# StanfordASL/GuSTO.jl

Hardware: AMD Instinct MI355X
Metric: converged trajectories/sec (batched SCP), freeflyer_se2 N=50, inputs resident in HBM (higher is better)
Workload: dtype f64

## Files before the change

gusto.jl_amd/csrc/common.hpp:

```cpp
#pragma once
#include <hip/hip_runtime.h>
#include <math.h>
#include <stdint.h>

#include "gusto_hip.h"

namespace gusto {

#define GD __device__ __forceinline__
typedef double v4d __attribute__((ext_vector_type(4)));

constexpr int ROW_HARD = 0;
constexpr int ROW_PEN = 1;
constexpr int ROW_PEN_TR = 2;
constexpr int ROW_PEN_EQ = 3;
constexpr int ROW_HARD_EQ = 4;
constexpr int ROW_EQ = 5;
GD bool row_is_hard(int kind) { return kind == ROW_HARD || kind == ROW_HARD_EQ; }

constexpr int RS_T = 0, RS_LAM = 1, RS_LAMB = 2, RS_S = 3, RS_DT = 4, RS_DL = 5, RS_DS = 6, RS_KA = 7, RS_KB = 8,
              RS_NVAR = 9;

#ifndef GUSTO_DUBINS_WAVES
#define GUSTO_DUBINS_WAVES 2
#endif
#ifndef GUSTO_WAVES_PER_EU
#define GUSTO_WAVES_PER_EU 1
#endif

#ifndef GUSTO_TO_SWEEP_CALL
#define GUSTO_TO_SWEEP_CALL true
#endif
#ifndef GUSTO_TO4_SWEEP_CALL
// ... 3 lines not shown
#define GUSTO_SWEEP_DPP 1
#endif
#ifndef GUSTO_FACTOR_LDS
#define GUSTO_FACTOR_LDS 1
#endif
#ifndef GUSTO_FACTOR_LDS_MV
#define GUSTO_FACTOR_LDS_MV 1
#endif
#ifndef GUSTO_FACTOR_LDS_HUU
#define GUSTO_FACTOR_LDS_HUU 0
#endif
#ifndef GUSTO_FACTOR_LDS_ROWS
#define GUSTO_FACTOR_LDS_ROWS 1
#endif
#ifndef GUSTO_FACTOR_HUU_DPP
#define GUSTO_FACTOR_HUU_DPP 0
#endif
#ifndef GUSTO_FACTOR_LAZY_SINV
#define GUSTO_FACTOR_LAZY_SINV 1
#endif
#ifndef GUSTO_FACTOR_LAZY_D
#define GUSTO_FACTOR_LAZY_D 1
#endif
static_assert(!(GUSTO_FACTOR_LDS_HUU && GUSTO_FACTOR_HUU_DPP), "H_uu to the Cholesky through LDS or by DPP, not both");
static_assert(!GUSTO_FACTOR_LAZY_D || GUSTO_FACTOR_LAZY_SINV, "GUSTO_FACTOR_LAZY_D forms D from the L^-1 that GUSTO_FACTOR_LAZY_SINV stores");
#ifndef GUSTO_USE_MFMA
#define GUSTO_USE_MFMA true
#endif
constexpr int GUSTO_TO_FREEFLYER_SE2 = 4, GUSTO_TO_ASTROBEE_SE3 = 5, GUSTO_TO_ASTROBEE_SE3_MANIFOLD = 6;
constexpr double TRAJOPT_DEFECT_REG = 1e-4;
constexpr int RS_EARLIER = 0, RS_ROW = 1, RS_ROW_LANE = 2;
template <int MODEL> struct MT;
template <> struct MT<GUSTO_FREEFLYER_SE2> {
    static constexpr int NDEF = 0;
    static constexpr int n = 6, m = 3, WS = 2, NFIX = 3, NHU = 2;
    static constexpr int WAVES_PER_EU = GUSTO_WAVES_PER_EU;
    static constexpr int RS_FORM = RS_ROW;
    static constexpr bool SWEEP_CALL = false;
    static constexpr bool SWEEP_DPP = GUSTO_SWEEP_DPP;
    static constexpr bool FACTOR_LDS = GUSTO_FACTOR_LDS;
    static constexpr bool FACTOR_REC = true;
    static constexpr bool MFMA = false;
    static constexpr int SCHED_PROBE = 2;
    static constexpr int SCHED_SLICE = 4;
    static constexpr bool LTI = true, HAS_OBS = true;
    static constexpr bool PG2 = true;
    static constexpr int pg_r0(int c) { return c < 3 ? c : (c < 6 ? c - 3 : c - 6); }
    static constexpr int pg_r1(int c) { return c < 3 ? c + 3 : (c < 6 ? c : c - 3); }
    static constexpr bool Anz(int i, int j) { return j == i + 3; }
    static constexpr bool Mnz(int i, int j) { return i == j || j == i + 3; }
    static constexpr bool Bnz(int i, int j) { return i == j + 3; }
    static constexpr bool Gnz(int i, int j) { return i == j || i == j + 3; }
    static constexpr bool Hnz(int, int) { return true; }
};
template <> struct MT<GUSTO_DUBINS_CAR> {
    static constexpr int NDEF = 0;
    static constexpr int n = 3, m = 1, WS = 2, NFIX = 6, NHU = 2;
    static constexpr int WAVES_PER_EU = GUSTO_DUBINS_WAVES;
    static constexpr int RS_FORM = RS_ROW;
    static constexpr bool SWEEP_CALL = false;
// ... 155 lines not shown
        for (int i2 = 0; i2 < n; i2++)
            for (int l2 = 0; l2 < n; l2++)
                if (T::Mnz(l2, i2) && (i2 < i || (i2 == i && l2 < l))) c++;
        return c;
    }
    static constexpr int NPHI = pos_phi(0, n);
    static constexpr int pos_gam(int l, int j) {
        int c = NPHI;
        for (int l2 = 0; l2 < n; l2++)
            for (int j2 = 0; j2 < m; j2++)
                if (T::Gnz(l2, j2) && (l2 < l || (l2 == l && j2 < j))) c++;
        return c;
    }
    static constexpr int NS = pos_gam(n, 0);
    static constexpr int S = (NS + 15) / 16 * 16;
    static constexpr bool USE = T::MFMA && T::NDEF == 0;
};

template <int MODEL> constexpr int rs_stride_rt(int N) { return MT<MODEL>::RS_FORM == RS_EARLIER ? N : (N + 63) & ~63; }
template <int MODEL, bool ONE> GD int rs_stride(int N) {
    if constexpr (ONE && MT<MODEL>::RS_FORM != RS_EARLIER) return 64;
    else return rs_stride_rt<MODEL>(N);
}
template <int MODEL, bool ONE> constexpr int rs_form() { return (ONE && MT<MODEL>::RS_FORM == RS_ROW_LANE) ? RS_ROW : MT<MODEL>::RS_FORM; }

struct WsLayout {
    int nslot;
    size_t rowstate, obs_nh, obs_c0, obs_mask, PG, PGS, QQ, Paft, Piaft, KD, Phicl, pvt, to_traj, total;
};
template <int MODEL> inline WsLayout make_ws_layout(int N, int n_obs) {
    using T = MT<MODEL>;
    constexpr int n = T::n, m = T::m, NZ = n + m;
    WsLayout L;
    L.nslot = T::NFIX + n_obs + 2 * n + T::NHU;
    size_t o = 0;
    auto take = [&](size_t c) { size_t r = o; o += (c + 1) & ~size_t(1); return r; };
    L.rowstate = take((size_t)RS_NVAR * L.nslot * rs_stride_rt<MODEL>(N));
    L.obs_nh = take((size_t)n_obs * T::WS * N);
    L.obs_c0 = take((size_t)n_obs * N);
    L.obs_mask = take((size_t)N);
    L.PG = take((size_t)(T::LTI ? 1 : N) * n * NZ);
    L.PGS = take(SpPG<MODEL>::USE ? (size_t)N * SpPG<MODEL>::S : 0);
    using R = Rec<MODEL>;
    L.QQ = take((size_t)N * R::SQQ);
    L.Paft = take((size_t)(N + 1) * R::SNN) + R::SNN;
    L.Piaft = take((size_t)(N + 1) * R::SNN) + R::SNN;
    L.KD = take((size_t)N * R::SKD);
// ... 451 lines not shown
```

gusto.jl_amd/csrc/ipm.hpp:

```cpp
#pragma once
#include "rows.hpp"

#ifndef GUSTO_COOP_CHOL_MIN
#define GUSTO_COOP_CHOL_MIN 7
#endif

namespace gusto {

extern __shared__ __attribute__((aligned(16))) double gusto_dyn_lds[];

template <int MODEL> constexpr bool costate_adjoint();

struct IpmOut {
    int status, iters;
    double obj, res_p, res_d, mu;
};

template <bool ONEWAVE> GD void blk_sync() {
    if constexpr (ONEWAVE) {
#ifdef GUSTO_STRICT_SYNC
        asm volatile("s_waitcnt vmcnt(0) lgkmcnt(0)\n\ts_barrier" ::: "memory");
#endif
        __builtin_amdgcn_fence(__ATOMIC_ACQ_REL, "wavefront");
        __builtin_amdgcn_wave_barrier();
// ... 318 lines not shown
                    for (int l = 0; l < n; l++) if (T::Bnz(l, j)) s += M[i * n + l] * (h * B[l * m + j]);
                    const double v = knot0 ? h * B[i * m + j] : 2.0 * s;
                    pg[i * NZ + n + j] = v;
                    if constexpr (SPR) if (T::Gnz(i, j)) ps[SP::pos_gam(i, j)] = v;
                }
                if constexpr (T::NDEF > 0) {
#pragma unroll
                    for (int j = 0; j < T::NDEF; j++) pg[i * NZ + n + (m - T::NDEF) + j] = (i == j) ? 1.0 : 0.0;
                }
            }
        }
        uint64_t mask = 0;
        if constexpr (T::HAS_OBS) {
            double xw[T::WS];
#pragma unroll
            for (int j = 0; j < T::WS; j++) xw[j] = xp[j];
            const Env E = K.env();
            for (int i = 0; i < E.n_obs; i++) {
                double nh[T::WS];
                const double dist = signed_distance<T::WS>(K.P, E, 0, xw, i, nh);
                if (dist < toggle) {
                    mask |= (uint64_t)1 << i;
                    double c0 = K.P.mp.clearance - dist;
#pragma unroll
                    for (int j = 0; j < T::WS; j++) {
                        K.obs_nh[((size_t)i * T::WS + j) * K.N + k] = nh[j];
                        c0 += nh[j] * xw[j];
                    }
                    K.obs_c0[(size_t)i * K.N + k] = c0;
                }
            }
        }
        K.obs_mask[k] = mask;
    }
    K.sync();
}

template <int MODEL, class BLK> GD void factor_sweep_mw(BLK& K, double* fail, Prof& pf) {
    using T = MT<MODEL>;
    using R = Rec<MODEL>;
    constexpr int n = T::n, m = T::m, NZ = n + m, NQ = NZ * (NZ + 1) / 2, NPG = n * NZ;
    constexpr int QPT = (NQ + 63) / 64, PPT = (NPG + 63) / 64;
    const int tid = K.tid, NT = K.nt(), N = K.N;
    for (int e = tid; e < n * n; e += NT) { K.sP[e] = 0; K.sPi[e] = 0; K.sGd[e] = 0; }
    double qq[QPT], pgn[PPT];
#pragma unroll
// ... 1776 lines not shown
        RowPre<NP> pre;
        if constexpr (NP > 0) {
            const int slot_u = RowSlots<MODEL>::ctl(K.P.n_obs);
            pre.load(rs, T::NFIX, slot_u, [&](int var) {
                return var == RS_T || var == RS_LAM || var == RS_S || var == RS_LAMB || (pass && (var == RS_KA || var == RS_KB));
            });
        }
        double hdx[ADJ ? n : 1];
#pragma unroll
        for (int i = 0; i < (ADJ ? n : 1); i++) hdx[i] = 0;
        OpStep<NP, ADJ, RS> op{rs, dxs, dus, pass, mu_t, tau, gAx, gAu, gBx, gBu, &pre, hdx};
        ctx.tick(0);
#if GUSTO_SEG_W2
        if constexpr (NCH > 0) {
            const bool cs = pass == 1 || ncomp == 0;
            segw_post_rows<MODEL, NCH>(K, cs ? SEGW_STEP_CS : SEGW_STEP, (double)pass, ctx.kappa, ctx.omega, ctx.Delta, mu_t, tau);
            RowCtx<MODEL> cm = ctx;
            cm.mask = (cs && NCH == 2) ? (cm.mask & seg_obs_share(0, 2)) : 0;
            visit_rows<MODEL>(cm, xs, us, op);
            segw_join();
            segw_rows_step_add<MODEL, NCH>(K.lds, K.P.ll.seg, k, (cs && NCH > 2) ? 1 : 0, op, gAx, gBx);
        } else
#endif
        visit_rows<MODEL>(ctx, xs, us, op);
        ctx.tick(3);
        if constexpr (ADJ) {
            if (adj_rt && k >= 1 && (pass == 1 || ncomp == 0)) {
                double Mk[n * n], Gamk[n * m], w[n];
                load_M_Gam(K, k, Mk, Gamk);
#pragma unroll
                for (int i = 0; i < n; i++) {
                    double s = hdx[i] + (pass ? K.gAx_(k, i) + mu_t * K.gBx_(k, i) : 0.0);
                    if (k == N - 1 && K.is_goal(i)) s += mugn[i];
                    w[i] = s;
                }
#pragma unroll
                for (int i = 0; i < n; i++) {
                    double s = 0;
#pragma unroll
                    for (int l = 0; l < n; l++) if (T::Mnz(l, i)) s += Mk[l * n + i] * w[l];
                    K.nun[k * n + i] = s;
                }
            }
        }
        l_amax = op.amax.value(); l_c0 = op.c0; l_c1 = op.c1; l_c2 = op.c2;
        if (pass == 0) {
#pragma unroll
// ... 85 lines not shown
        constexpr int NP = (n <= 8 && T::NDEF == 0) ? T::NFIX + T::NHU : 0;
        RowPre<NP> pre;
        if constexpr (NP > 0) {
            const int slot_u = RowSlots<MODEL>::ctl(K.P.n_obs);
            const bool upd = alpha_prev != 0.0;
            pre.load(rs, T::NFIX, slot_u, [&](int var) {
                return var == RS_T || var == RS_LAM || var == RS_S || var == RS_LAMB ||
                       (upd && (var == RS_DT || var == RS_DL || var == RS_DS));
            });
        }
        constexpr bool LRTR = MODEL == GUSTO_ASTROBEE_SE3;
        OpResidHess<n, m, NP, LRTR, RS> op{rs, Hx, Hu, rdx, rdu, gx0, gu0, alpha_prev, &pre};
        ctx.tick(0);
#if GUSTO_SEG_W2
        if constexpr (NCH > 0) {
            segw_post_rows<MODEL, NCH>(K, SEGW_ROWS_R, alpha_prev, ctx.kappa, ctx.omega, ctx.Delta, 0.0, 0.0);
            RowCtx<MODEL> cm = ctx;
            cm.mask = 0;
            visit_rows<MODEL>(cm, xs, us, op);
            segw_join();
            segw_rows_resid_add<MODEL, NCH>(K.lds, K.P.ll.seg, k, NCH - 1, op, Hx, rdx, gx0);
        } else
#endif
        visit_rows<MODEL>(ctx, xs, us, op);
        ctx.tick(3);
#pragma unroll
        for (int i = 0; i < n; i++) K.dXs_(k, i) = gx0[i];
#pragma unroll
        for (int i = 0; i < m; i++) K.dUs_(k, i) = gu0[i];
        l_comp = op.comp;
        l_resp = nanmax(l_resp, op.maxrp);
#pragma unroll
        for (int i = 0; i < m; i++) {
            const double wi_ = (i < m - T::NDEF) ? wk : TRAJOPT_DEFECT_REG * wk;
            Hu[sidx(i, i, m)] += 2 * wi_; rdu[i] += 2 * wi_ * us[i];
        }
        {
            double vs[n], vd[n];
#pragma unroll
            for (int i = 0; i < n; i++) {
                const double n1 = (k + 1 < N) ? K.nu[(k + 1) * n + i] : 0.0, n0 = (k >= 1) ? K.nu[k * n + i] : 0.0;
                vs[i] = n1 + n0; vd[i] = n1 - n0;
                l_numax = fmax(l_numax, fabs(K.nu[k * n + i]));
            }
#pragma unroll
            for (int i = 0; i < n; i++) {
                double s = vd[i];
// ... 154 lines not shown
    RS rs{K.rowstate, K.P.wl.nslot, rs_stride<MODEL, BLK::ONE>(N), act ? k : 0};
#define GUSTO_REFRESH_K()                                     \
    do {                                                      \
        asm volatile("" : "+v"(k));                           \
        ctx.k = k; rs.k = act ? k : 0;                        \
        ctx.xp = K.Xp + (act ? k : 0) * n;                    \
    } while (0)

    auto load_iter = [&](double* xs, double* us) {
#pragma unroll
        for (int i = 0; i < n; i++) xs[i] = K.Xw[k * n + i];
#pragma unroll
        for (int i = 0; i < m; i++) us[i] = K.Uw[k * m + i];
    };

    double ncomp_l = 0;
    if (act) {
        double xs[n], us[m];
#pragma unroll
        for (int i = 0; i < n; i++) { xs[i] = (k == 0) ? K.x_init[i] : K.Xp[k * n + i]; K.Xw[k * n + i] = xs[i]; K.nu[k * n + i] = 0; }
#pragma unroll
        for (int i = 0; i < m; i++) { us[i] = K.Up[k * m + i]; K.Uw[k * m + i] = us[i]; }
        OpInit<RS> op{rs, muw};
        visit_rows<MODEL>(ctx, xs, us, op);
        ncomp_l = op.ncomp;
    }
    if (k == 0) {
        *fail = 0.0;
        for (int i = 0; i < n; i++) { mug[i] = 0; mugn[i] = 0; }
    }
    const double ncomp = block_reduce<BLK::ONE>(ncomp_l, OpSum(), red);
    K.sync();
    pf.tick(PF_INIT);

    constexpr bool LINC = BLK::C::LC_LDS;
    if constexpr (LINC) {
        if (act) {
            double xpk[n], c2[2];
#pragma unroll
            for (int i = 0; i < n; i++) xpk[i] = K.Xp[k * n + i];
            Dyn<MODEL>::lin_cache(K.P.mp, xpk, c2);
            K.lcl[2 * k] = c2[0]; K.lcl[2 * k + 1] = c2[1];
        }
        K.sync();
    }
    int status = GUSTO_SOLVER_FAILED, it = 0, n_acc = 0;
    bool adj_ok = true;
// ... 240 lines not shown
                xs[i] += alpha * K.dXs_(k, i);
                K.Xw[k * n + i] = xs[i];
                K.nu[k * n + i] += alpha * (K.nun[k * n + i] - K.nu[k * n + i]);
            }
#pragma unroll
            for (int i = 0; i < m; i++) { us[i] += alpha * K.dUs_(k, i); K.Uw[k * m + i] = us[i]; }
        }
        alpha_prev = alpha;
        if constexpr (n > 4) {
            if (k < n) mug[k] += alpha * (mugn[k] - mug[k]);
        } else if (k == 0) {
            for (int i = 0; i < n; i++) mug[i] += alpha * (mugn[i] - mug[i]);
        }
        K.sync();
        pf.tick(PF_UPDATE);
    }
    double l_obj = 0;
    if (act) {
        double xs[n], us[m];
        load_iter(xs, us);
#pragma unroll
        for (int i = 0; i < m; i++) l_obj += ((i < m - T::NDEF) ? wk : TRAJOPT_DEFECT_REG * wk) * us[i] * us[i];
        OpSlackSum<RS> op{rs};
        visit_rows<MODEL>(ctx, xs, us, op);
        l_obj += op.sum;
    }
    const double obj = block_reduce<BLK::ONE>(l_obj, OpSum(), red);
    K.sync();
#undef GUSTO_REFRESH_K
    out.status = status; out.iters = it; out.obj = obj / kappa; out.res_p = res_p; out.res_d = res_d; out.mu = mu;
}

}
```

gusto.jl_amd/csrc/launch.hpp:

```cpp
#pragma once
#include <algorithm>
#include <cstdlib>
#include <cstdio>
#include <cstring>

#include "handle.hpp"
#include "scp.hpp"

using namespace gusto;

#ifdef GUSTO_DEV_KNOBS
static inline const char* dev_env(const char* k) { return getenv(k); }
#else
static inline const char* dev_env(const char*) { return nullptr; }
#endif

static inline int launch_waves(gusto_handle h) {
    int w = h->waves;
    if (const char* e = dev_env("GUSTO_DEV_WAVES")) w = atoi(e);
    const int need = (h->N + 63) / 64;
    return std::min(4, std::max(w, need));
}
template <int MODEL> static int fill_params(gusto_handle h, KParams& P, int B, bool need_env = true) {
    using T = MT<MODEL>;
    memset(&P, 0, sizeof(P));
    P.N = h->N; P.B = B; P.n_fresh = B;
    if (!fill_env(h, P, T::HAS_OBS, need_env)) {
        h->err = "gusto_set_env_batch described a different number of problems than gusto_set_problems";
        return GUSTO_ERR_STATE;
    }
    P.hist_cap = h->hist_cap;
    P.sp = h->sp; P.mp = h->mp; P.io = h->io;
    warm_defaults(MODEL, P.io);
    P.X = h->d_X; P.U = h->d_U;
    P.x_init = h->d_xinit; P.goal_lo = h->d_glo; P.goal_hi = h->d_ghi; P.tf = h->d_tf;
    P.sub_Delta = h->d_subD; P.sub_omega = h->d_subW; P.sub_toggle = h->d_subT; P.sub_X = h->d_subX; P.sub_U = h->d_subU;
    P.sub_obj = h->d_subObj; P.sub_status = h->d_subSt; P.sub_iters = h->d_subIt;
    P.st_i = h->d_sti; P.st_d = h->d_std;
    P.J_true = h->d_Jt; P.J_full = h->d_Jf; P.conv = h->d_conv; P.Delta = h->d_Delta; P.omega = h->d_omega; P.rho = h->d_rho;
    P.accept = h->d_acc; P.scp_status = h->d_scp; P.solver_status = h->d_sol; P.tr_sat = h->d_tr; P.cvx_sat = h->d_cvx;
    P.ipm_it = h->d_ipm;
    P.tp = h->tp; P.to_mu = h->d_to_mu; P.to_xtol = h->d_to_xtol; P.to_ftol = h->d_to_ftol; P.to_ctol = h->d_to_ctol;
    P.wl = make_ws_layout<MODEL>(h->N, P.n_obs);
    P.ll = make_lds_layout<MODEL>(h->N, launch_waves(h) > (h->N + 63) / 64);
    HIPCHK(h, h->d_queue.alloc(SQ_WORDS));
#ifdef GUSTO_PROFILE
    HIPCHK(h, h->d_prof.alloc((size_t)h->batch_cap * PROF_N));
#endif
    P.prof = h->d_prof;
    return GUSTO_OK;
}

template <class Kern, class Pre>
static int enqueue_solve(gusto_handle h, KParams& P, Kern kern, dim3 grid, dim3 block, size_t lds, Pre pre) {
    HIPCHK(h, h->d_ws.ensure(P.wl.total * (size_t)grid.x));
    P.ws = h->d_ws;
    HIPCHK(h, hipEventRecord(h->ev0, h->stream));
    { int rc = pre(); if (rc) return rc; }
    hipLaunchKernelGGL(kern, grid, block, lds, h->stream, P);
    HIPCHK(h, hipGetLastError());
    HIPCHK(h, hipEventRecord(h->ev1, h->stream));
    h->sched_err = 0;
    HIPCHK(h, gusto_fetch_sched_err(h));
    h->pending = true;
    return GUSTO_OK;
}

template <int MODEL> static int launch_scp(gusto_handle h, int mode, int max_iter, int force) {
    using T = MT<MODEL>;
    KParams P;
    int rc = fill_params<MODEL>(h, P, h->B);
    if (rc) return rc;
    P.mode = mode; P.max_iter = max_iter; P.force = force;
    const int NT = 64 * launch_waves(h);
    size_t lds = (size_t)P.ll.total * sizeof(double);
    if (const char* pad = dev_env("GUSTO_DEV_LDS_KB")) lds = std::max(lds, (size_t)atoi(pad) * 1024);
    if (lds > 160 * 1024) { h->err = "problem does not fit the 160 KiB LDS of a CU"; return GUSTO_ERR_ARG; }
    auto kern = (NT == 64) ? &scp_kernel<MODEL, true> : &scp_kernel<MODEL, false>;
    int per_cu = 0, cus = 0;
// ... 109 lines not shown
```

gusto.jl_amd/csrc/rows.hpp:

```cpp
#pragma once
#include <type_traits>

#include "models.hpp"

namespace gusto {

#ifndef GUSTO_OBS_BATCH
#define GUSTO_OBS_BATCH 4
#endif
constexpr int OBS_BATCH = GUSTO_OBS_BATCH, FX_OBS = 64;

template <int CNT> struct RowEv {
    double g;
    double raw;
    double gr[CNT];
    double hd[CNT];
};

template <int MODEL> struct RowCtx {
    const KParams* P;
    int N, k, nslot;
    double kappa, omega, Delta;
    GPtr<const double> xp;
    uint64_t mask;
// ... 38 lines not shown
template <bool ISU, int I0, int CNT, int FX = -1, class Op>
GD void lin_row(Op& op, int slot, int kind, const double* v, const double* b, double c0, double mul, double off) {
    RowEv<CNT> ev;
    double g = c0;
#pragma unroll
    for (int j = 0; j < CNT; j++) {
        g += b[j] * v[I0 + j];
        ev.gr[j] = mul * b[j];
        ev.hd[j] = 0.0;
    }
    ev.raw = g;
    ev.g = mul * g - off;
    op.template row<ISU, I0, CNT, FX>(slot, kind, ev);
}

template <int MODEL> struct RowSlots {
    using T = MT<MODEL>;
    static constexpr bool CT = T::RS_FORM != RS_EARLIER;
    GD static int ctl(int n_obs) { return CT ? T::NFIX : T::NFIX + n_obs + 2 * T::n; }
    GD static int goal(int n_obs) { return CT ? T::NFIX + T::NHU : T::NFIX + n_obs; }
    GD static int obs(int n_obs) { return CT ? T::NFIX + T::NHU + 2 * T::n : T::NFIX; }
};

template <int MODEL, class Op> GD void visit_obs_rows(const RowCtx<MODEL>& c, const double* xs, Op& op, uint64_t mk) {
    using T = MT<MODEL>;
    const double kw = c.kappa * c.omega;
    const int slot_obs = RowSlots<MODEL>::obs(c.P->n_obs);
    while (mk) {
        int oi[OBS_BATCH], oslot[OBS_BATCH];
        bool ov[OBS_BATCH];
        int last = 0;
#pragma unroll
        for (int q = 0; q < OBS_BATCH; q++) {
            ov[q] = mk != 0;
            if (ov[q]) { last = __ffsll((unsigned long long)mk) - 1; mk &= mk - 1; }
            oi[q] = last; oslot[q] = slot_obs + last;
        }
        double ob[OBS_BATCH][T::WS], oc[OBS_BATCH];
#pragma unroll
        for (int q = 0; q < OBS_BATCH; q++) {
#pragma unroll
            for (int j = 0; j < T::WS; j++) ob[q][j] = -(c.obs_nh + (size_t)(oi[q] * T::WS + j) * (size_t)c.N)[c.k];
            oc[q] = (c.obs_c0 + (size_t)oi[q] * (size_t)c.N)[c.k];
        }
        op.obs_load(oslot);
        static_for<0, OBS_BATCH>([&](auto Q) {
            constexpr int q = decltype(Q)::value;
            if (ov[q]) lin_row<false, 0, T::WS, FX_OBS + q>(op, oslot[q], ROW_PEN, xs, ob[q], oc[q], kw, 0.0);
        });
    }
}

template <int MODEL, class Op> GD void visit_ctl_rows(const RowCtx<MODEL>& c, const double* us, Op& op) {
    using T = MT<MODEL>;
    constexpr int n = T::n;
    constexpr bool is2 = MODEL == GUSTO_FREEFLYER_SE2, FB = Op::FIX_BATCH;
    const gusto_model_params& mp = c.P->mp;
    const int slot_u = RowSlots<MODEL>::ctl(c.P->n_obs);
    if (c.k < c.N - 1) {
        constexpr int nf = is2 ? 2 : 3, im = is2 ? 2 : 3, nm = is2 ? 1 : 3;
        double af[nf], am[nm];
#pragma unroll
        for (int j = 0; j < nf; j++) af[j] = 1.0 / (mp.mass * mp.mass);
#pragma unroll
        for (int j = 0; j < nm; j++) { const double ji = 1.0 / mp.Jdiag[is2 ? 2 : j]; am[j] = ji * ji; }
        if constexpr (FB) {
            int fs[OBS_BATCH];
#pragma unroll
            for (int q = 0; q < OBS_BATCH; q++) fs[q] = slot_u + (q < 1 ? 0 : 1);
            op.obs_load(fs);
        }
        quad_row<true, 0, nf, (FB ? FX_OBS + 0 : T::NFIX)>(op, slot_u, ROW_HARD, us, af, nullptr, -mp.hard_limit_accel * mp.hard_limit_accel,
                              1.0 / (mp.hard_limit_accel * mp.hard_limit_accel), 0.0);
        quad_row<true, im, nm, (FB ? FX_OBS + 1 : T::NFIX + 1)>(op, slot_u + 1, ROW_HARD, us, am, nullptr, -mp.hard_limit_alpha * mp.hard_limit_alpha,
                               1.0 / (mp.hard_limit_alpha * mp.hard_limit_alpha), 0.0);
    }
}

template <int MODEL, class Op> GD void visit_rows(const RowCtx<MODEL>& c, const double* xs, const double* us, Op& op) {
    using T = MT<MODEL>;
    constexpr int n = T::n;
    const gusto_model_params& mp = c.P->mp;
    const double kw = c.kappa * c.omega;
    const int slot_obs = RowSlots<MODEL>::obs(c.P->n_obs), slot_goal = RowSlots<MODEL>::goal(c.P->n_obs), slot_u = RowSlots<MODEL>::ctl(c.P->n_obs);
    double one[n];
#pragma unroll
    for (int j = 0; j < n; j++) one[j] = 1.0;

    if constexpr (T::NDEF > 0) {
        constexpr bool is2 = MODEL == GUSTO_TO_FREEFLYER_SE2, man = MODEL == GUSTO_TO_ASTROBEE_SE3_MANIFOLD;
        constexpr int nv = is2 ? 2 : 3, iw = is2 ? 5 : (man ? 10 : 9), nw = is2 ? 1 : 3, m0 = T::m - T::NDEF;
        constexpr bool FB = Op::FIX_BATCH;
#define GUSTO_FXQ(q) (FB ? FX_OBS + (q) : -1)
        auto batch = [&](int s0, int s1, int s2, int s3) {
            if constexpr (FB) { const int fs[OBS_BATCH] = {s0, s1, s2, s3}; op.obs_load(fs); }
        };
        static_assert(OBS_BATCH == 4 || !FB, "batches of four rows");
        if constexpr (!man) {
            batch(0, 1, 2, 2);
            quad_row<false, 0, n, GUSTO_FXQ(0)>(op, 0, ROW_HARD, xs, one, c.xp, -c.Delta, 1.0 / c.Delta, 0.0);
        } else {
            const double* qp = c.xp + 6;
// ... 80 lines not shown
#define GUSTO_FXB(i, fx) ((FB && (i) < NB1) ? FX_OBS + (i) : (fx))
        if constexpr (FB) {
            int fs[OBS_BATCH];
#pragma unroll
            for (int q = 0; q < OBS_BATCH; q++) fs[q] = q < NB1 ? q : NB1 - 1;
            op.obs_load(fs);
        }
        if constexpr (!man) {
            quad_row<false, 0, n, GUSTO_FXB(0, 0)>(op, slot++, ROW_PEN_TR, xs, one, c.xp, 0.0, kw, c.kappa * c.Delta);
        } else {
            const double* qp = c.xp + 6;
            const double qn = sqrt(qp[0] * qp[0] + qp[1] * qp[1] + qp[2] * qp[2] + qp[3] * qp[3]);
            double bp[4], bm[4], c0 = qn - 1.0;
#pragma unroll
            for (int j = 0; j < 4; j++) { bp[j] = qp[j] / qn; bm[j] = -bp[j]; c0 -= qp[j] * qp[j] / qn; }
            lin_row<false, 6, 4, GUSTO_FXB(0, 0)>(op, slot++, ROW_HARD_EQ, xs, bm, -c0, kw, c.kappa * c.P->sp.eps);
            lin_row<false, 6, 4, GUSTO_FXB(1, 1)>(op, slot++, ROW_PEN_EQ, xs, bp, c0, kw, c.kappa * c.P->sp.eps);
            const double m1 = -1.0;
            lin_row<false, 6, 1, GUSTO_FXB(2, 2)>(op, slot++, ROW_PEN, xs, &m1, 0.0, kw, 0.0);
        }
        quad_row<false, 3, nv, GUSTO_FXB(T::NFIX - 2, T::NFIX - 2)>(op, slot++, ROW_PEN, xs, one, nullptr, -mp.hard_limit_vel * mp.hard_limit_vel, kw, 0.0);
        quad_row<false, iw, nw, GUSTO_FXB(T::NFIX - 1, T::NFIX - 1)>(op, slot++, ROW_PEN, xs, one, nullptr, -mp.hard_limit_omega * mp.hard_limit_omega, kw, 0.0);
        c.tick(1);
        visit_obs_rows<MODEL>(c, xs, op, c.mask);
        c.tick(2);
        if (!c.skip_ctl) visit_ctl_rows<MODEL>(c, us, op);
#undef GUSTO_FXB
    } else {
        static_for<0, n>([&](auto I) {
            constexpr int i = decltype(I)::value;
            const double p1 = 1.0, m1 = -1.0;
            lin_row<false, i, 1, i>(op, i, ROW_PEN, xs, &p1, -mp.x_max[i], kw, 0.0);
            lin_row<false, i, 1, n + i>(op, n + i, ROW_PEN, xs, &m1, mp.x_min[i], kw, 0.0);
        });
        if (c.k < c.N - 1) {
            const double p1 = 1.0, m1 = -1.0;
            lin_row<true, 0, 1, T::NFIX>(op, slot_u, ROW_HARD, us, &p1, -mp.u_max, 1.0 / fabs(mp.u_max), 0.0);
            lin_row<true, 0, 1, T::NFIX + 1>(op, slot_u + 1, ROW_HARD, us, &m1, mp.u_min, 1.0 / fabs(mp.u_min), 0.0);
        }
    }
    if (c.boxmask != 0 && c.k == c.N - 1) {
        static_assert(OBS_BATCH >= 4, "a batch holds the four rows of two coordinates");
        static_for<0, (n + 1) / 2>([&](auto G) {
            constexpr int i0 = 2 * decltype(G)::value, i1 = (i0 + 1 < n) ? i0 + 1 : i0;
            if ((c.boxmask >> i0) & 3u) {
                const double lo0 = c.goal_lo[i0], hi0 = c.goal_hi[i0], lo1 = c.goal_lo[i1], hi1 = c.goal_hi[i1];
                int oslot[OBS_BATCH];
#pragma unroll
                for (int q = 0; q < OBS_BATCH; q++) oslot[q] = slot_goal + 2 * ((q < 2) ? i0 : i1) + (q & 1);
                op.obs_load(oslot);
                const double p1 = 1.0, m1 = -1.0;
                if (lo0 != hi0) {
                    const double hw = (isfinite(hi0) && isfinite(lo0)) ? 0.5 * (hi0 - lo0) : 1.0;
                    const double sc = 1.0 / fmax(1e-3, fmin(1.0, hw));
                    if (isfinite(hi0)) lin_row<false, i0, 1, FX_OBS + 0>(op, oslot[0], ROW_HARD, xs, &p1, -hi0, sc, 0.0);
                    if (isfinite(lo0)) lin_row<false, i0, 1, FX_OBS + 1>(op, oslot[1], ROW_HARD, xs, &m1, lo0, sc, 0.0);
                }
                if (i1 != i0 && lo1 != hi1) {
                    const double hw = (isfinite(hi1) && isfinite(lo1)) ? 0.5 * (hi1 - lo1) : 1.0;
                    const double sc = 1.0 / fmax(1e-3, fmin(1.0, hw));
                    if (isfinite(hi1)) lin_row<false, i1, 1, FX_OBS + 2>(op, oslot[2], ROW_HARD, xs, &p1, -hi1, sc, 0.0);
                    if (isfinite(lo1)) lin_row<false, i1, 1, FX_OBS + 3>(op, oslot[3], ROW_HARD, xs, &m1, lo1, sc, 0.0);
                }
            }
        });
    }
}

template <int FORM> struct RowState {
    GPtr<double> base;
    int nslot, kp, k;
    GD auto& at(int var, int slot) const {
        if constexpr (FORM == RS_EARLIER) return (base + (size_t)(var * nslot + slot) * (size_t)kp)[k];
        else {
            typedef __attribute__((address_space(1))) char GC;
            typedef __attribute__((address_space(1))) double GV;
            const int mid = FORM == RS_ROW_LANE ? var : RS_NVAR / 2;
            GC* r = (GC*)base.p + (size_t)(((unsigned)(slot * RS_NVAR + mid) * (unsigned)kp + (unsigned)k) * 8u);
            return *(GV*)(r + (ptrdiff_t)((var - mid) * kp) * 8);
        }
    }
};

template <int NP> struct RowPre {
    double v[RS_NVAR][NP > 0 ? NP : 1];
    template <class RS, class F> GD void load(const RS& rs, int nfix, int slot_u, F&& want) {
#pragma unroll
        for (int var = 0; var < RS_NVAR; var++)
#pragma unroll
            for (int i = 0; i < NP; i++)
                if (want(var)) v[var][i] = rs.at(var, i < nfix ? i : slot_u + (i - nfix));
    }
};

struct ObsPre {
    double v[RS_NVAR][OBS_BATCH];
    template <class RS, class F> GD void load(const RS& rs, const int* slot, F&& want) {
#pragma unroll
        for (int var = 0; var < RS_NVAR; var++)
            if (want(var)) {
#pragma unroll
                for (int q = 0; q < OBS_BATCH; q++) v[var][q] = rs.at(var, slot[q]);
            }
    }
};

template <class RS> struct OpInit {
    static constexpr bool FIX_BATCH = false;
    RS rs;
    double muw;
    int ncomp = 0;
    GD void obs_load(const int*) {}
    template <bool ISU, int I0, int CNT, int FX> GD void row(int slot, int kind, const RowEv<CNT>& ev) {
        if (kind == ROW_EQ) {
            rs.at(RS_T, slot) = 1.0; rs.at(RS_LAM, slot) = 0.0; rs.at(RS_LAMB, slot) = 0.0; rs.at(RS_S, slot) = 0.0;
        } else if (row_is_hard(kind)) {
            const double t = fmax(-ev.g, 1e-2), mu0 = (muw > 0) ? muw : 0.01;
            rs.at(RS_T, slot) = t; rs.at(RS_LAM, slot) = mu0 / t; rs.at(RS_LAMB, slot) = 0.0; rs.at(RS_S, slot) = 0.0;
            ncomp += 1;
        } else if (muw > 0) {
            const double g = ev.g, ag = fabs(g), rr = sqrt(g * g + 4 * muw * muw);
            const double big = muw + 0.5 * (rr + ag), small = muw + 2 * muw * muw / (rr + ag);
            const double s = (g >= 0) ? big : small, t = (g >= 0) ? small : big;
            rs.at(RS_S, slot) = s; rs.at(RS_T, slot) = t; rs.at(RS_LAM, slot) = muw / t; rs.at(RS_LAMB, slot) = muw / s;
            ncomp += 2;
        } else {
            const double s = fmax(ev.g, 0.0) + 0.01;
            rs.at(RS_S, slot) = s; rs.at(RS_T, slot) = s - ev.g; rs.at(RS_LAM, slot) = 0.5; rs.at(RS_LAMB, slot) = 0.5;
            ncomp += 2;
        }
    }
};

template <int n, int m, int NP, bool LRTR, class RS> struct OpResidHess {
    static constexpr bool FIX_BATCH = NP == 0;
    RS rs;
// ... 2 lines not shown
    const RowPre<NP>* pre;
    double comp = 0, maxrp = 0;
    ObsPre ob;
    double trs = 0, trg[LRTR ? n : 1], trh[LRTR ? n : 1];
    GD void obs_load(const int* slot) {
        const bool upd = alpha_prev != 0.0;
        ob.load(rs, slot, [&](int var) {
            return var == RS_T || var == RS_LAM || var == RS_S || var == RS_LAMB ||
                   (upd && (var == RS_DT || var == RS_DL || var == RS_DS));
        });
    }
    template <int FX> GD double get(int var, int slot) const {
        if constexpr (FX >= FX_OBS) return ob.v[var][FX - FX_OBS];
        else if constexpr (FX >= 0 && NP > 0) return pre->v[var][FX];
        else return rs.at(var, slot);
    }
    template <bool ISU, int I0, int CNT, int FX> GD void row(int slot, int kind, const RowEv<CNT>& ev) {
        double t = get<FX>(RS_T, slot), lam = get<FX>(RS_LAM, slot);
        double sig, rp;
        if (alpha_prev != 0.0) {
            const double dl = get<FX>(RS_DL, slot);
            t += alpha_prev * get<FX>(RS_DT, slot);
            lam += alpha_prev * dl;
            rs.at(RS_T, slot) = t; rs.at(RS_LAM, slot) = lam;
        }
        if (kind == ROW_EQ) {
            rp = ev.g;
            sig = 1.0 / TRAJOPT_EQ_DELTA;
        } else if (row_is_hard(kind)) {
            rp = ev.g + t;
            comp += t * lam;
            sig = lam * rcp_nr(t);
        } else {
            double s = get<FX>(RS_S, slot), lamb = get<FX>(RS_LAMB, slot);
            if (alpha_prev != 0.0) {
                s += alpha_prev * get<FX>(RS_DS, slot);
                lamb -= alpha_prev * get<FX>(RS_DL, slot);
                rs.at(RS_S, slot) = s; rs.at(RS_LAMB, slot) = lamb;
            }
            rp = ev.g - s + t;
            comp += t * lam + s * lamb;
            sig = lam * lamb * rcp_nr(t * lamb + lam * s);
        }
        maxrp = nanmax(maxrp, fabs(rp));
        double* H = ISU ? Hu : Hx;
        double* r = ISU ? rdu : rdx;
        double* g0 = ISU ? gu0 : gx0;
        const double coef0 = lam + sig * ev.g;
        constexpr int dim = ISU ? m : n;
        if constexpr (LRTR && !ISU && CNT == n) {
            trs = sig;
#pragma unroll
            for (int a = 0; a < CNT; a++) {
                r[I0 + a] += lam * ev.gr[a];
                g0[I0 + a] += coef0 * ev.gr[a];
                trg[a] = ev.gr[a];
                trh[a] = lam * ev.hd[a];
            }
            return;
        }
#pragma unroll
// ... 29 lines not shown
    StepFrac amax;
    double c0 = 0, c1 = 0, c2 = 0;
    ObsPre ob;
    GD void obs_load(const int* slot) {
        ob.load(rs, slot, [&](int var) {
            return var == RS_T || var == RS_LAM || var == RS_S || var == RS_LAMB || (pass && (var == RS_KA || var == RS_KB));
        });
    }
    template <int FX> GD double get(int var, int slot) const {
        if constexpr (FX >= FX_OBS) return ob.v[var][FX - FX_OBS];
        else if constexpr (FX >= 0 && NP > 0) return pre->v[var][FX];
        else return rs.at(var, slot);
    }
    template <bool ISU, int I0, int CNT, int FX> GD void row(int slot, int kind, const RowEv<CNT>& ev) {
        const double t = get<FX>(RS_T, slot), lam = get<FX>(RS_LAM, slot);
        const double ka = pass ? get<FX>(RS_KA, slot) : 0.0;
        const double* dv = ISU ? dus : dxs;
        double w = 0;
#pragma unroll
        for (int a = 0; a < CNT; a++) w += ev.gr[a] * dv[I0 + a];
        double dt, dl, ds;
        double cA = 0, cB = 0;
        double sig = 0;
        if (kind == ROW_EQ) {
            sig = 1.0 / TRAJOPT_EQ_DELTA;
            dl = sig * (ev.g + w);
            if constexpr (HDX && !ISU) {
                const double sw = sig * w;
#pragma unroll
                for (int a = 0; a < CNT; a++) hdx[I0 + a] += sw * ev.gr[a];
            }
            if (pass == 0) {
                rs.at(RS_KA, slot) = 0.0;
                const double cE = lam + sig * ev.g;
                double* gA = ISU ? gAu : gAx;
#pragma unroll
                for (int a = 0; a < CNT; a++) gA[I0 + a] += cE * ev.gr[a];
            }
            if (pass) { rs.at(RS_DT, slot) = 0.0; rs.at(RS_DL, slot) = dl; rs.at(RS_DS, slot) = 0.0; }
            return;
        }
        if (row_is_hard(kind)) {
            const double rp = ev.g + t;
            const double rt = rcp_nr(t);
            dt = -rp - w;
            dl = (mu_t - t * lam - ka - lam * dt) * rt;
            ds = 0.0;
            if (pass == 0) { cA = (lam * rp - dt * dl) * rt; cB = rt; }
            if constexpr (HDX) sig = lam * rt;
        } else {
            const double s = get<FX>(RS_S, slot), lamb = get<FX>(RS_LAMB, slot);
            const double kb = pass ? get<FX>(RS_KB, slot) : 0.0;
            const double rp = ev.g - s + t;
            const double il = rcp_nr(lamb), lol = lam * il;
            const double D = t + lol * s;
            const double rho0 = mu_t - t * lam - ka + lam * rp - lol * (mu_t - s * lamb - kb);
            const double rD = rcp_nr(D);
            dl = (rho0 + lam * w) * rD;
            ds = (mu_t - s * lamb - kb + s * dl) * il;
            dt = -rp - w + ds;
            if constexpr (HDX) sig = lam * rD;
            amax.test(s, ds, tau);
            amax.test(lamb, -dl, tau);
            if (pass == 0) {
                c0 += s * lamb; c1 += ds * lamb - s * dl; c2 -= ds * dl; rs.at(RS_KB, slot) = -ds * dl;
                cA = lam + (lam * rp - t * lam - dt * dl + lol * (s * lamb - ds * dl)) * rD;
                cB = (1.0 - lol) * rD;
            }
        }
        if constexpr (HDX && !ISU) {
            const double sw = sig * w;
#pragma unroll
            for (int a = 0; a < CNT; a++) hdx[I0 + a] += sw * ev.gr[a] + (lam * ev.hd[a]) * dv[I0 + a];
        }
        amax.test(t, dt, tau);
        amax.test(lam, dl, tau);
        if (pass == 0) {
            c0 += t * lam; c1 += dt * lam + t * dl; c2 += dt * dl; rs.at(RS_KA, slot) = dt * dl;
            double* gA = ISU ? gAu : gAx;
            double* gB = ISU ? gBu : gBx;
#pragma unroll
            for (int a = 0; a < CNT; a++) { gA[I0 + a] += cA * ev.gr[a]; gB[I0 + a] += cB * ev.gr[a]; }
        }
        if (pass) { rs.at(RS_DT, slot) = dt; rs.at(RS_DL, slot) = dl; rs.at(RS_DS, slot) = ds; }
    }
};

template <class RS> struct OpSlackSum {
    static constexpr bool FIX_BATCH = false;
    RS rs;
    double sum = 0;
    GD void obs_load(const int*) {}
    template <bool ISU, int I0, int CNT, int FX> GD void row(int slot, int kind, const RowEv<CNT>&) {
        if (!row_is_hard(kind) && kind != ROW_EQ) sum += rs.at(RS_S, slot);
    }
};

struct OpCheck {
    static constexpr bool FIX_BATCH = false;
    double eps;
    bool ok = true;
    GD void obs_load(const int*) {}
    template <bool ISU, int I0, int CNT, int FX> GD void row(int, int kind, const RowEv<CNT>& ev) {
        if (ISU) return;
        if (kind == ROW_PEN && ev.raw >= eps) ok = false;
        if (kind == ROW_PEN_EQ && (ev.raw <= -eps || ev.raw >= eps)) ok = false;
// ... 5 lines not shown
```

gusto.jl_amd/csrc/scp.hpp:

```cpp
#pragma once
#include "ipm.hpp"

#ifndef GUSTO_WAVES_PER_EU
#define GUSTO_WAVES_PER_EU 1
#endif

namespace gusto {

template <class BLK> GD double cost_true(BLK& K, const double* U) {
    constexpr int m = BLK::m, mc = m - BLK::T::NDEF;
    const int k = K.tid;
    double l = 0;
    if (k >= 1 && k < K.N) {
#pragma unroll
        for (int j = 0; j < mc; j++) l += 0.5 * K.dt * (U[(k - 1) * m + j] * U[(k - 1) * m + j] + U[k * m + j] * U[k * m + j]);
    }
    return block_reduce<BLK::ONE>(l, OpSum(), K.misc);
}

template <int MODEL, class BLK> GD double trust_region_ratio(BLK& K, const double* X, const double* U, const double* Xp, const double* Up) {
    using T = MT<MODEL>;
    constexpr int n = T::n, m = T::m;
    const int k = K.tid, N = K.N;
    double num = 0, den = 0;
// ... 105 lines not shown
        const int h = n_hist;
        if (tid == 0) { P.solver_status[hb + h] = io.status; P.ipm_it[hb + h] = io.iters; }
        if (io.status != GUSTO_SOLVER_OPTIMAL && io.status != GUSTO_SOLVER_ALMOST) {
            stop = GUSTO_STOP_SUBPROBLEM_FAILED;
            break;
        }
        double dn = 0, xn = 0;
        bool cvx_l = true;
        if (k < N) {
            double xs[n], us[m];
#pragma unroll
            for (int i = 0; i < n; i++) {
                xs[i] = K.Xw[k * n + i];
                const double e = xs[i] - K.Xp[k * n + i];
                dn += e * e; xn += xs[i] * xs[i];
            }
#pragma unroll
            for (int i = 0; i < m; i++) us[i] = K.Uw[k * m + i];
            RowCtx<MODEL> ctx;
            ctx.P = &P; ctx.N = N; ctx.k = k; ctx.nslot = P.wl.nslot; ctx.kappa = 1.0; ctx.omega = 1.0; ctx.Delta = 1.0;
            ctx.xp = K.Xp + k * n; ctx.mask = K.obs_mask[k]; ctx.obs_nh = K.obs_nh; ctx.obs_c0 = K.obs_c0;
            ctx.goal_lo = K.goal_lo; ctx.goal_hi = K.goal_hi; ctx.boxmask = K.boxmask;
            OpCheck op{sp.eps};
            visit_rows<MODEL>(ctx, xs, us, op);
            cvx_l = op.ok;
        }
        tk(1);
        const double max_d2 = block_reduce<ONEWAVE>(dn, OpMax(), K.misc);
        const double max_x2 = block_reduce<ONEWAVE>(xn, OpMax(), K.misc);
        const double conv = sqrt(max_d2) / sqrt(max_x2);
        const int cvx_sat = block_reduce<ONEWAVE>(cvx_l ? 0.0 : 1.0, OpMax(), K.misc) == 0.0;
        tk(2);
        const int tr_sat = (max_d2 - Delta <= P.io.tr_tol * fmax(1.0, Delta));
        int accept, status;
        double Delta_n, omega_n;
        if (tr_sat) {
            const double rho = trust_region_ratio<MODEL>(K, K.Xw, K.Uw, K.Xp, K.Up);
            tk(3);
            if (tid == 0) P.rho[hb + n_rho] = rho;
            n_rho++;
            if (rho > sp.rho1) {
                status = GUSTO_SCP_INACCURATE_MODEL; accept = 0; Delta_n = sp.beta_fail * Delta; omega_n = omega;
            } else {
                accept = 1;
                Delta_n = (rho < sp.rho0) ? fmin(sp.beta_succ * Delta, sp.Delta0) : Delta;
                if (!cvx_sat) { status = GUSTO_SCP_VIOLATES_CONSTRAINTS; omega_n = sp.gamma_fail * omega; }
                else { status = GUSTO_SCP_OK; omega_n = omega; }
// ... 464 lines not shown
```

Before: 151,900.

## Interleave row-state variables into 16-byte pairs for wide global loads/stores

Adds an RS_PAIR row-state layout for single-wave blocks that interleaves related IPM variables (t/lam, s/lamb, dt/dl, ka/kb) so each pair is read or written with one 16-byte vector access. All row-state accessors (init, residual, step, prefetch) gain pair paths, and KB is now stored together with KA. An optional paired obstacle-normal layout is added but disabled by default. Alignment checks are added at launch. The aim is fewer global memory instructions per row, in exchange for more code paths and a changed memory layout.

```diff
diff --git a/gusto.jl_amd/csrc/common.hpp b/gusto.jl_amd/csrc/common.hpp
--- a/gusto.jl_amd/csrc/common.hpp
+++ b/gusto.jl_amd/csrc/common.hpp
@@ -3,12 +3,15 @@
 #include <math.h>
 #include <stdint.h>
 
+#include <type_traits>
+
 #include "gusto_hip.h"
 
 namespace gusto {
 
 #define GD __device__ __forceinline__
 typedef double v4d __attribute__((ext_vector_type(4)));
+typedef double v2d __attribute__((ext_vector_type(2)));
 
 constexpr int ROW_HARD = 0;
 constexpr int ROW_PEN = 1;
@@ -58,6 +61,12 @@
 #ifndef GUSTO_FACTOR_LAZY_D
 #define GUSTO_FACTOR_LAZY_D 1
 #endif
+#ifndef GUSTO_RS_PAIR
+#define GUSTO_RS_PAIR 1
+#endif
+#ifndef GUSTO_OBS_NH_PAIR
+#define GUSTO_OBS_NH_PAIR 0
+#endif
 static_assert(!(GUSTO_FACTOR_LDS_HUU && GUSTO_FACTOR_HUU_DPP), "H_uu to the Cholesky through LDS or by DPP, not both");
 static_assert(!GUSTO_FACTOR_LAZY_D || GUSTO_FACTOR_LAZY_SINV, "GUSTO_FACTOR_LAZY_D forms D from the L^-1 that GUSTO_FACTOR_LAZY_SINV stores");
 #ifndef GUSTO_USE_MFMA
@@ -65,13 +74,19 @@
 #endif
 constexpr int GUSTO_TO_FREEFLYER_SE2 = 4, GUSTO_TO_ASTROBEE_SE3 = 5, GUSTO_TO_ASTROBEE_SE3_MANIFOLD = 6;
 constexpr double TRAJOPT_DEFECT_REG = 1e-4;
-constexpr int RS_EARLIER = 0, RS_ROW = 1, RS_ROW_LANE = 2;
+constexpr int RS_EARLIER = 0, RS_ROW = 1, RS_ROW_LANE = 2, RS_PAIR = 3;
+constexpr int RS_NPAIR = 4, RS_PAIR_KP = 64;
+constexpr int RS_PAIR_A[RS_NPAIR] = {RS_T, RS_S, RS_DT, RS_KA}, RS_PAIR_B[RS_NPAIR] = {RS_LAM, RS_LAMB, RS_DL, RS_KB};
+constexpr int rs_pair_plane(int var) { return var == RS_T || var == RS_LAM ? 0 : (var == RS_S || var == RS_LAMB ? 1 : (var == RS_DT || var == RS_DL ? 2 : (var == RS_KA || var == RS_KB ? 3 : -1))); }
+constexpr int rs_pair_half(int var) { return (var == RS_LAM || var == RS_LAMB || var == RS_DL || var == RS_KB) ? 1 : 0; }
 template <int MODEL> struct MT;
 template <> struct MT<GUSTO_FREEFLYER_SE2> {
     static constexpr int NDEF = 0;
     static constexpr int n = 6, m = 3, WS = 2, NFIX = 3, NHU = 2;
     static constexpr int WAVES_PER_EU = GUSTO_WAVES_PER_EU;
     static constexpr int RS_FORM = RS_ROW;
+    static constexpr bool RS_PAIRS = GUSTO_RS_PAIR;
+    static constexpr bool OBS_NH_PAIR = GUSTO_OBS_NH_PAIR;
     static constexpr bool SWEEP_CALL = false;
     static constexpr bool SWEEP_DPP = GUSTO_SWEEP_DPP;
     static constexpr bool FACTOR_LDS = GUSTO_FACTOR_LDS;
@@ -273,7 +288,15 @@
     if constexpr (ONE && MT<MODEL>::RS_FORM != RS_EARLIER) return 64;
     else return rs_stride_rt<MODEL>(N);
 }
-template <int MODEL, bool ONE> constexpr int rs_form() { return (ONE && MT<MODEL>::RS_FORM == RS_ROW_LANE) ? RS_ROW : MT<MODEL>::RS_FORM; }
+template <int MODEL, class = void> struct rs_pair_trait { static constexpr bool value = false; };
+template <int MODEL> struct rs_pair_trait<MODEL, std::void_t<decltype(MT<MODEL>::RS_PAIRS)>> { static constexpr bool value = MT<MODEL>::RS_PAIRS; };
+template <int MODEL, class = void> struct nh_pair_trait { static constexpr bool value = false; };
+template <int MODEL> struct nh_pair_trait<MODEL, std::void_t<decltype(MT<MODEL>::OBS_NH_PAIR)>> { static constexpr bool value = MT<MODEL>::OBS_NH_PAIR; };
+template <int MODEL, bool ONE> constexpr int rs_form() {
+    if (ONE && rs_pair_trait<MODEL>::value) return RS_PAIR;
+    return (ONE && MT<MODEL>::RS_FORM == RS_ROW_LANE) ? RS_ROW : MT<MODEL>::RS_FORM;
+}
+template <int MODEL, bool ONE> constexpr bool obs_nh_pair() { return ONE && MT<MODEL>::WS == 2 && nh_pair_trait<MODEL>::value; }
 
 struct WsLayout {
     int nslot;
diff --git a/gusto.jl_amd/csrc/ipm.hpp b/gusto.jl_amd/csrc/ipm.hpp
--- a/gusto.jl_amd/csrc/ipm.hpp
+++ b/gusto.jl_amd/csrc/ipm.hpp
@@ -364,6 +364,12 @@
                 if (dist < toggle) {
                     mask |= (uint64_t)1 << i;
                     double c0 = K.P.mp.clearance - dist;
+                    if constexpr (obs_nh_pair<MODEL, BLK::ONE>()) {
+                        typedef __attribute__((address_space(1))) v2d GP;
+                        *(GP*)((K.obs_nh + (size_t)i * 2 * K.N).p + 2 * k) = v2d{nh[0], nh[1]};
+#pragma unroll
+                        for (int j = 0; j < T::WS; j++) c0 += nh[j] * xw[j];
+                    } else
 #pragma unroll
                     for (int j = 0; j < T::WS; j++) {
                         K.obs_nh[((size_t)i * T::WS + j) * K.N + k] = nh[j];
@@ -2186,7 +2192,7 @@
             segw_rows_step_add<MODEL, NCH>(K.lds, K.P.ll.seg, k, (cs && NCH > 2) ? 1 : 0, op, gAx, gBx);
         } else
 #endif
-        visit_rows<MODEL>(ctx, xs, us, op);
+        visit_rows<MODEL, obs_nh_pair<MODEL, BLK::ONE>()>(ctx, xs, us, op);
         ctx.tick(3);
         if constexpr (ADJ) {
             if (adj_rt && k >= 1 && (pass == 1 || ncomp == 0)) {
@@ -2318,7 +2324,7 @@
             segw_rows_resid_add<MODEL, NCH>(K.lds, K.P.ll.seg, k, NCH - 1, op, Hx, rdx, gx0);
         } else
 #endif
-        visit_rows<MODEL>(ctx, xs, us, op);
+        visit_rows<MODEL, obs_nh_pair<MODEL, BLK::ONE>()>(ctx, xs, us, op);
         ctx.tick(3);
 #pragma unroll
         for (int i = 0; i < n; i++) K.dXs_(k, i) = gx0[i];
@@ -2519,7 +2525,7 @@
 #pragma unroll
         for (int i = 0; i < m; i++) { us[i] = K.Up[k * m + i]; K.Uw[k * m + i] = us[i]; }
         OpInit<RS> op{rs, muw};
-        visit_rows<MODEL>(ctx, xs, us, op);
+        visit_rows<MODEL, obs_nh_pair<MODEL, BLK::ONE>()>(ctx, xs, us, op);
         ncomp_l = op.ncomp;
     }
     if (k == 0) {
@@ -2806,7 +2812,7 @@
 #pragma unroll
         for (int i = 0; i < m; i++) l_obj += ((i < m - T::NDEF) ? wk : TRAJOPT_DEFECT_REG * wk) * us[i] * us[i];
         OpSlackSum<RS> op{rs};
-        visit_rows<MODEL>(ctx, xs, us, op);
+        visit_rows<MODEL, obs_nh_pair<MODEL, BLK::ONE>()>(ctx, xs, us, op);
         l_obj += op.sum;
     }
     const double obj = block_reduce<BLK::ONE>(l_obj, OpSum(), red);
diff --git a/gusto.jl_amd/csrc/launch.hpp b/gusto.jl_amd/csrc/launch.hpp
--- a/gusto.jl_amd/csrc/launch.hpp
+++ b/gusto.jl_amd/csrc/launch.hpp
@@ -43,6 +43,7 @@
     P.tp = h->tp; P.to_mu = h->d_to_mu; P.to_xtol = h->d_to_xtol; P.to_ftol = h->d_to_ftol; P.to_ctol = h->d_to_ctol;
     P.wl = make_ws_layout<MODEL>(h->N, P.n_obs);
     P.ll = make_lds_layout<MODEL>(h->N, launch_waves(h) > (h->N + 63) / 64);
+    if (P.wl.rowstate % 2 || P.wl.obs_nh % 2 || P.wl.total % 2) { h->err = "workspace layout: row state or obstacle normals not 16-byte aligned"; return GUSTO_ERR_STATE; }
     HIPCHK(h, h->d_queue.alloc(SQ_WORDS));
 #ifdef GUSTO_PROFILE
     HIPCHK(h, h->d_prof.alloc((size_t)h->batch_cap * PROF_N));
@@ -55,6 +56,7 @@
 static int enqueue_solve(gusto_handle h, KParams& P, Kern kern, dim3 grid, dim3 block, size_t lds, Pre pre) {
     HIPCHK(h, h->d_ws.ensure(P.wl.total * (size_t)grid.x));
     P.ws = h->d_ws;
+    if ((uintptr_t)P.ws % 16) { h->err = "workspace not 16-byte aligned"; return GUSTO_ERR_STATE; }
     HIPCHK(h, hipEventRecord(h->ev0, h->stream));
     { int rc = pre(); if (rc) return rc; }
     hipLaunchKernelGGL(kern, grid, block, lds, h->stream, P);
diff --git a/gusto.jl_amd/csrc/rows.hpp b/gusto.jl_amd/csrc/rows.hpp
--- a/gusto.jl_amd/csrc/rows.hpp
+++ b/gusto.jl_amd/csrc/rows.hpp
@@ -84,7 +84,7 @@
     GD static int obs(int n_obs) { return CT ? T::NFIX + T::NHU + 2 * T::n : T::NFIX; }
 };
 
-template <int MODEL, class Op> GD void visit_obs_rows(const RowCtx<MODEL>& c, const double* xs, Op& op, uint64_t mk) {
+template <int MODEL, bool NHP = false, class Op> GD void visit_obs_rows(const RowCtx<MODEL>& c, const double* xs, Op& op, uint64_t mk) {
     using T = MT<MODEL>;
     const double kw = c.kappa * c.omega;
     const int slot_obs = RowSlots<MODEL>::obs(c.P->n_obs);
@@ -99,6 +99,16 @@
             oi[q] = last; oslot[q] = slot_obs + last;
         }
         double ob[OBS_BATCH][T::WS], oc[OBS_BATCH];
+        if constexpr (NHP) {
+            static_assert(T::WS == 2, "a pair of doubles");
+            typedef __attribute__((address_space(1))) const v2d GP;
+#pragma unroll
+            for (int q = 0; q < OBS_BATCH; q++) {
+                const v2d nh = *(GP*)((c.obs_nh + (size_t)oi[q] * 2 * (size_t)c.N).p + 2 * c.k);
+                ob[q][0] = -nh.x; ob[q][1] = -nh.y;
+                oc[q] = (c.obs_c0 + (size_t)oi[q] * (size_t)c.N)[c.k];
+            }
+        } else
 #pragma unroll
         for (int q = 0; q < OBS_BATCH; q++) {
 #pragma unroll
@@ -139,7 +149,7 @@
     }
 }
 
-template <int MODEL, class Op> GD void visit_rows(const RowCtx<MODEL>& c, const double* xs, const double* us, Op& op) {
+template <int MODEL, bool NHP = false, class Op> GD void visit_rows(const RowCtx<MODEL>& c, const double* xs, const double* us, Op& op) {
     using T = MT<MODEL>;
     constexpr int n = T::n;
     const gusto_model_params& mp = c.P->mp;
@@ -266,7 +276,7 @@
         quad_row<false, 3, nv, GUSTO_FXB(T::NFIX - 2, T::NFIX - 2)>(op, slot++, ROW_PEN, xs, one, nullptr, -mp.hard_limit_vel * mp.hard_limit_vel, kw, 0.0);
         quad_row<false, iw, nw, GUSTO_FXB(T::NFIX - 1, T::NFIX - 1)>(op, slot++, ROW_PEN, xs, one, nullptr, -mp.hard_limit_omega * mp.hard_limit_omega, kw, 0.0);
         c.tick(1);
-        visit_obs_rows<MODEL>(c, xs, op, c.mask);
+        visit_obs_rows<MODEL, NHP>(c, xs, op, c.mask);
         c.tick(2);
         if (!c.skip_ctl) visit_ctl_rows<MODEL>(c, us, op);
 #undef GUSTO_FXB
@@ -311,12 +321,27 @@
     }
 }
 
-template <int FORM> struct RowState {
+template <int FORM_> struct RowState {
+    static constexpr int FORM = FORM_;
     GPtr<double> base;
     int nslot, kp, k;
+    static constexpr unsigned PSLOT = RS_NVAR * RS_PAIR_KP * 8u, PMID = 2u * RS_PAIR_KP * 16u;
+    GD auto& pair(int pl, int slot) const {
+        static_assert(FORM == RS_PAIR, "pairs exist in RS_PAIR only");
+        typedef __attribute__((address_space(1))) char GC;
+        typedef __attribute__((address_space(1))) v2d GP;
+        GC* r = (GC*)base.p + (size_t)((unsigned)slot * PSLOT + PMID + (unsigned)k * 16u);
+        return *(GP*)(r + (ptrdiff_t)((pl - 2) * RS_PAIR_KP * 16));
+    }
     GD auto& at(int var, int slot) const {
         if constexpr (FORM == RS_EARLIER) return (base + (size_t)(var * nslot + slot) * (size_t)kp)[k];
-        else {
+        else if constexpr (FORM == RS_PAIR) {
+            typedef __attribute__((address_space(1))) char GC;
+            typedef __attribute__((address_space(1))) double GV;
+            const int pl = rs_pair_plane(var);
+            GC* r = (GC*)base.p + (size_t)((unsigned)slot * PSLOT + PMID + (unsigned)k * (pl < 0 ? 8u : 16u));
+            return *(GV*)(r + (ptrdiff_t)(pl < 0 ? 2 * RS_PAIR_KP * 16 : (pl - 2) * RS_PAIR_KP * 16 + rs_pair_half(var) * 8));
+        } else {
             typedef __attribute__((address_space(1))) char GC;
             typedef __attribute__((address_space(1))) double GV;
             const int mid = FORM == RS_ROW_LANE ? var : RS_NVAR / 2;
@@ -329,6 +354,19 @@
 template <int NP> struct RowPre {
     double v[RS_NVAR][NP > 0 ? NP : 1];
     template <class RS, class F> GD void load(const RS& rs, int nfix, int slot_u, F&& want) {
+        if constexpr (RS::FORM == RS_PAIR) {
+#pragma unroll
+            for (int pl = 0; pl < RS_NPAIR; pl++)
+#pragma unroll
+                for (int i = 0; i < NP; i++)
+                    if (want(RS_PAIR_A[pl]) || want(RS_PAIR_B[pl])) {
+                        const v2d p = rs.pair(pl, i < nfix ? i : slot_u + (i - nfix));
+                        v[RS_PAIR_A[pl]][i] = p.x; v[RS_PAIR_B[pl]][i] = p.y;
+                    }
+#pragma unroll
+            for (int i = 0; i < NP; i++)
+                if (want(RS_DS)) v[RS_DS][i] = rs.at(RS_DS, i < nfix ? i : slot_u + (i - nfix));
+        } else
 #pragma unroll
         for (int var = 0; var < RS_NVAR; var++)
 #pragma unroll
@@ -340,6 +378,21 @@
 struct ObsPre {
     double v[RS_NVAR][OBS_BATCH];
     template <class RS, class F> GD void load(const RS& rs, const int* slot, F&& want) {
+        if constexpr (RS::FORM == RS_PAIR) {
+#pragma unroll
+            for (int pl = 0; pl < RS_NPAIR; pl++)
+                if (want(RS_PAIR_A[pl]) || want(RS_PAIR_B[pl])) {
+#pragma unroll
+                    for (int q = 0; q < OBS_BATCH; q++) {
+                        const v2d p = rs.pair(pl, slot[q]);
+                        v[RS_PAIR_A[pl]][q] = p.x; v[RS_PAIR_B[pl]][q] = p.y;
+                    }
+                }
+            if (want(RS_DS)) {
+#pragma unroll
+                for (int q = 0; q < OBS_BATCH; q++) v[RS_DS][q] = rs.at(RS_DS, slot[q]);
+            }
+        } else
 #pragma unroll
         for (int var = 0; var < RS_NVAR; var++)
             if (want(var)) {
@@ -356,6 +409,26 @@
     int ncomp = 0;
     GD void obs_load(const int*) {}
     template <bool ISU, int I0, int CNT, int FX> GD void row(int slot, int kind, const RowEv<CNT>& ev) {
+        if constexpr (RS::FORM == RS_PAIR) {
+            if (kind == ROW_EQ) {
+                rs.pair(0, slot) = v2d{1.0, 0.0}; rs.pair(1, slot) = v2d{0.0, 0.0};
+            } else if (row_is_hard(kind)) {
+                const double t = fmax(-ev.g, 1e-2), mu0 = (muw > 0) ? muw : 0.01;
+                rs.pair(0, slot) = v2d{t, mu0 / t}; rs.pair(1, slot) = v2d{0.0, 0.0};
+                ncomp += 1;
+            } else if (muw > 0) {
+                const double g = ev.g, ag = fabs(g), rr = sqrt(g * g + 4 * muw * muw);
+                const double big = muw + 0.5 * (rr + ag), small = muw + 2 * muw * muw / (rr + ag);
+                const double s = (g >= 0) ? big : small, t = (g >= 0) ? small : big;
+                rs.pair(1, slot) = v2d{s, muw / s}; rs.pair(0, slot) = v2d{t, muw / t};
+                ncomp += 2;
+            } else {
+                const double s = fmax(ev.g, 0.0) + 0.01;
+                rs.pair(1, slot) = v2d{s, 0.5}; rs.pair(0, slot) = v2d{s - ev.g, 0.5};
+                ncomp += 2;
+            }
+            return;
+        }
         if (kind == ROW_EQ) {
             rs.at(RS_T, slot) = 1.0; rs.at(RS_LAM, slot) = 0.0; rs.at(RS_LAMB, slot) = 0.0; rs.at(RS_S, slot) = 0.0;
         } else if (row_is_hard(kind)) {
@@ -404,7 +477,10 @@
             const double dl = get<FX>(RS_DL, slot);
             t += alpha_prev * get<FX>(RS_DT, slot);
             lam += alpha_prev * dl;
+            if constexpr (RS::FORM == RS_PAIR) rs.pair(0, slot) = v2d{t, lam};
+            else {
             rs.at(RS_T, slot) = t; rs.at(RS_LAM, slot) = lam;
+            }
         }
         if (kind == ROW_EQ) {
             rp = ev.g;
@@ -418,7 +494,10 @@
             if (alpha_prev != 0.0) {
                 s += alpha_prev * get<FX>(RS_DS, slot);
                 lamb -= alpha_prev * get<FX>(RS_DL, slot);
+                if constexpr (RS::FORM == RS_PAIR) rs.pair(1, slot) = v2d{s, lamb};
+                else {
                 rs.at(RS_S, slot) = s; rs.at(RS_LAMB, slot) = lamb;
+                }
             }
             rp = ev.g - s + t;
             comp += t * lam + s * lamb;
@@ -494,6 +573,7 @@
         double dt, dl, ds;
         double cA = 0, cB = 0;
         double sig = 0;
+        double kbn = 0.0;
         if (kind == ROW_EQ) {
             sig = 1.0 / TRAJOPT_EQ_DELTA;
             dl = sig * (ev.g + w);
@@ -503,12 +583,16 @@
                 for (int a = 0; a < CNT; a++) hdx[I0 + a] += sw * ev.gr[a];
             }
             if (pass == 0) {
+                if constexpr (RS::FORM == RS_PAIR) rs.pair(3, slot) = v2d{0.0, 0.0};
+                else
                 rs.at(RS_KA, slot) = 0.0;
                 const double cE = lam + sig * ev.g;
                 double* gA = ISU ? gAu : gAx;
 #pragma unroll
                 for (int a = 0; a < CNT; a++) gA[I0 + a] += cE * ev.gr[a];
             }
+            if constexpr (RS::FORM == RS_PAIR) { if (pass) { rs.pair(2, slot) = v2d{0.0, dl}; rs.at(RS_DS, slot) = 0.0; } }
+            else
             if (pass) { rs.at(RS_DT, slot) = 0.0; rs.at(RS_DL, slot) = dl; rs.at(RS_DS, slot) = 0.0; }
             return;
         }
@@ -535,7 +619,10 @@
             amax.test(s, ds, tau);
             amax.test(lamb, -dl, tau);
             if (pass == 0) {
-                c0 += s * lamb; c1 += ds * lamb - s * dl; c2 -= ds * dl; rs.at(RS_KB, slot) = -ds * dl;
+                c0 += s * lamb; c1 += ds * lamb - s * dl; c2 -= ds * dl;
+                if constexpr (RS::FORM == RS_PAIR) kbn = -ds * dl;
+                else
+                rs.at(RS_KB, slot) = -ds * dl;
                 cA = lam + (lam * rp - t * lam - dt * dl + lol * (s * lamb - ds * dl)) * rD;
                 cB = (1.0 - lol) * rD;
             }
@@ -548,12 +635,17 @@
         amax.test(t, dt, tau);
         amax.test(lam, dl, tau);
         if (pass == 0) {
-            c0 += t * lam; c1 += dt * lam + t * dl; c2 += dt * dl; rs.at(RS_KA, slot) = dt * dl;
+            c0 += t * lam; c1 += dt * lam + t * dl; c2 += dt * dl;
+            if constexpr (RS::FORM == RS_PAIR) rs.pair(3, slot) = v2d{dt * dl, kbn};
+            else
+            rs.at(RS_KA, slot) = dt * dl;
             double* gA = ISU ? gAu : gAx;
             double* gB = ISU ? gBu : gBx;
 #pragma unroll
             for (int a = 0; a < CNT; a++) { gA[I0 + a] += cA * ev.gr[a]; gB[I0 + a] += cB * ev.gr[a]; }
         }
+        if constexpr (RS::FORM == RS_PAIR) { if (pass) { rs.pair(2, slot) = v2d{dt, dl}; rs.at(RS_DS, slot) = ds; } }
+        else
         if (pass) { rs.at(RS_DT, slot) = dt; rs.at(RS_DL, slot) = dl; rs.at(RS_DS, slot) = ds; }
     }
 };
diff --git a/gusto.jl_amd/csrc/scp.hpp b/gusto.jl_amd/csrc/scp.hpp
--- a/gusto.jl_amd/csrc/scp.hpp
+++ b/gusto.jl_amd/csrc/scp.hpp
@@ -151,7 +151,7 @@
             ctx.xp = K.Xp + k * n; ctx.mask = K.obs_mask[k]; ctx.obs_nh = K.obs_nh; ctx.obs_c0 = K.obs_c0;
             ctx.goal_lo = K.goal_lo; ctx.goal_hi = K.goal_hi; ctx.boxmask = K.boxmask;
             OpCheck op{sp.eps};
-            visit_rows<MODEL>(ctx, xs, us, op);
+            visit_rows<MODEL, obs_nh_pair<MODEL, ONEWAVE>()>(ctx, xs, us, op);
             cvx_l = op.ok;
         }
         tk(1);
```

Result: faster. 157,800 (median of 6 runs) (+3.8%).
